# coin-or/Ipopt

Hardware: AMD Instinct MI355X
Metric: KKT factor+solve GFLOP/s (1 numeric LDL^T factorisation + 2 solves per Ipopt iteration) (higher is better)
Workload: dtype f64; 1 GPU; synth_1e6; kkt_dim=1000000, triplet_nnz=20143342, nnz_L=230755000, ordering=nested dissection + minimum-degree leaves (own), supernodes=50052, tree_levels=110, maxfront=3260, num_neg=400000

## Files before the change

### ipopt_amd/csrc/device_view.hip.inc

```
constexpr int FLAG_STRIDE = 32;

typedef double v2d __attribute__((ext_vector_type(2)));
struct DevView {
    const int* sn_colptr; const int* sn_rowptr; const int* sn_rows; const int* rel;
    const int* child_ptr; const int* child_idx; const int* sn_owner; const int* sn_parent; const int* col_owner;
    const long long* panel_off; const long long* cb_off; const long long* minv_off;
    const int* acolptr; const int* apos; const int* arow; const int* acol;
    const int* dup_ptr; const int* dup_src;
    const int* rslot_ptr; const int* rslot_idx; const int* rslot_col; int rslot_len;
    const int* level_sn;
    const FrontMeta* fmeta;
    const int* relinv;
    const GroupLink* gtab;
    const int* tile_tab;
    const ChildMeta* cmeta;
    const int* perm;
    const double* tvals;
    double* aval;
    double* scale;
    double* scale2;
    double* arv;
    unsigned long long* rowmax;
    double* L;
    double* cb;
    double* wbuf;
    double* minv;
    double* dinv; double* doff; int* ptype; int* lperm;
    int4*   fstat;
    double* xw;
    double* cvec;
    double* bw; double* xacc;
    double* gpart;
    double* zb;
    double* ybuf;
    double* arena; const long long* arena_off;
    double* top_rhs; const long long* top_rhs_off;
    double pivtol, pivtol2, small;
    int* colfail;
    int* qstat;
    double* cnorm;
    const ChainLink* chlink; const ChainDesc* chdesc;
    int strace_b;
    unsigned long long* strace;
    const int* chwg_f; const int* chwg_b; const int* chwait; int* sflag_t; int* sflag_dot; double* dpart; v2d* ytag; v2d* xtag;
    int xcd_affine;
    int* apfail;
    int* tcnt;
    double* isg; int* hasis;
    const int* lc_ptr; const LeafLink* lc_link;
    int* sflag_s;
    v2d* cbt; const long long* cbt_off;
    int* sflag_p;
    int* sflag_b; int* sflag_d; int* sepoch;
    int* zpiv;
    int n, nnz_a, nsn, rank;
    int fastpiv;
    double fastu;
    int asm_pull;
    int norestore;
    unsigned long long* dbg;
};

template <int CTRL>
__device__ __forceinline__ double dpp_f64(double x)
{
    int lo = __double2loint(x), hi = __double2hiint(x);
    lo = __builtin_amdgcn_update_dpp(lo, lo, CTRL, 0xF, 0xF, false);
    hi = __builtin_amdgcn_update_dpp(hi, hi, CTRL, 0xF, 0xF, false);
    return __hiloint2double(hi, lo);
}
__device__ __forceinline__ double readlane_f64(double x, int l)
{
    return __hiloint2double(__builtin_amdgcn_readlane(__double2hiint(x), l), __builtin_amdgcn_readlane(__double2loint(x), l));
}
__device__ __forceinline__ double wave_max_all(double x)
{
    x = fmax(x, dpp_f64<0xB1>(x));
    x = fmax(x, dpp_f64<0x4E>(x));
    x = fmax(x, dpp_f64<0x141>(x));
    x = fmax(x, dpp_f64<0x140>(x));
    return fmax(fmax(readlane_f64(x, 0), readlane_f64(x, 16)), fmax(readlane_f64(x, 32), readlane_f64(x, 48)));
}
__device__ __forceinline__ unsigned long long wave_or_all(unsigned long long v)
{
    int lo = (int)(v & 0xffffffffull), hi = (int)(v >> 32);
    lo |= __builtin_amdgcn_update_dpp(lo, lo, 0xB1, 0xF, 0xF, false);  hi |= __builtin_amdgcn_update_dpp(hi, hi, 0xB1, 0xF, 0xF, false);
    lo |= __builtin_amdgcn_update_dpp(lo, lo, 0x4E, 0xF, 0xF, false);  hi |= __builtin_amdgcn_update_dpp(hi, hi, 0x4E, 0xF, 0xF, false);
    lo |= __builtin_amdgcn_update_dpp(lo, lo, 0x141, 0xF, 0xF, false); hi |= __builtin_amdgcn_update_dpp(hi, hi, 0x141, 0xF, 0xF, false);
    lo |= __builtin_amdgcn_update_dpp(lo, lo, 0x140, 0xF, 0xF, false); hi |= __builtin_amdgcn_update_dpp(hi, hi, 0x140, 0xF, 0xF, false);
    const unsigned int l = (unsigned)(__builtin_amdgcn_readlane(lo, 0) | __builtin_amdgcn_readlane(lo, 16) | __builtin_amdgcn_readlane(lo, 32) | __builtin_amdgcn_readlane(lo, 48));
    const unsigned int h = (unsigned)(__builtin_amdgcn_readlane(hi, 0) | __builtin_amdgcn_readlane(hi, 16) | __builtin_amdgcn_readlane(hi, 32) | __builtin_amdgcn_readlane(hi, 48));
    return ((unsigned long long)h << 32) | l;
}
__device__ __forceinline__ double wave_sum_dpp(double x)
{
    x += dpp_f64<0xB1>(x);
    x += dpp_f64<0x4E>(x);
    x += dpp_f64<0x141>(x);
    x += dpp_f64<0x140>(x);
    return (readlane_f64(x, 0) + readlane_f64(x, 16)) + (readlane_f64(x, 32) + readlane_f64(x, 48));
}
__device__ __forceinline__ double wave_sum(double x)
{
#pragma unroll
    for (int off = 32; off >= 1; off >>= 1) x += __shfl_xor(x, off);
    return x;
}
```

### ipopt_amd/csrc/kernels_solve.hip.inc

```
__global__ void k_load_rhs(DevView V, const double* b)
{
    for (int i = blockIdx.x * blockDim.x + threadIdx.x; i < V.n; i += gridDim.x * blockDim.x) V.xw[i] = V.scale[i] * b[V.perm[i]];
}
__global__ void k_store_sol(DevView V, double* b)
{
    for (int i = blockIdx.x * blockDim.x + threadIdx.x; i < V.n; i += gridDim.x * blockDim.x) b[V.perm[i]] = V.scale[i] * V.xw[i];
}

__global__ void k_refine_residual(DevView V, int first)
{
    for (int i = blockIdx.x * blockDim.x + threadIdx.x; i < V.n; i += gridDim.x * blockDim.x)
        V.xacc[i] = first ? V.xw[i] : V.xacc[i] + V.xw[i];
}
__global__ void k_refine_spmv(DevView V)
{
    for (int i = blockIdx.x * blockDim.x + threadIdx.x; i < V.n; i += gridDim.x * blockDim.x) {
        double acc = 0.0;
        for (int p = V.rslot_ptr[i]; p < V.rslot_ptr[i + 1]; ++p) {
            const int q = V.rslot_idx[p];
            const int r = V.arow[q], c = V.acol[q];
            acc += V.aval[q] * V.xacc[r == i ? c : r];
        }
        V.xw[i] = V.bw[i] - acc;
    }
// ... 1147 lines not shown
        flag_raise(&V.sflag_dot[(size_t)(C.dot0 + r) * FLAG_STRIDE], epoch);
        if (tr && tid == 0) tr[3] = wall_clock64();
        return;
    }
    const int jt = r - ndots;
    const int j = C.nlinks - 1 - jt;
    const int nlater = jt;
    const ChainLink Me = uni(V.chlink[C.link0 + j]);
    const int k = Me.k, c0 = Me.c0;
    double mreg[16], lrA[16], lrB[16];
    int lpv = 0;
    auto fetch_block = [&](double (&lr)[16], const int i) {
        const ChainLink L = V.chlink[C.link0 + C.nlinks - 1 - i];
        const double* Lb = V.L + uni(Me.panel_off) + (uni(L.koff) - uni(Me.koff));
        const int kl = uni(L.k);
        const int off = (col < k ? col : 0) * uni(Me.ldp) + part;
#pragma unroll
        for (int u = 0; u < 16; ++u) lr[u] = (col < k && part + 4 * u < kl) ? Lb[off + 4 * u] : 0.0;
    };
    if (!poller) {
        const double* Mg = V.minv + Me.minv_off;
#pragma unroll
        for (int u = 0; u < 16; ++u) { const int q = col + part + 4 * u; mreg[u] = (col < k && q < k) ? Mg[q + (size_t)col * k] : 0.0; }
        if (col < k) lpv = V.lperm[c0 + col];
        if (nlater > 0) fetch_block(lrA, 0);
        if (nlater > 1) fetch_block(lrB, 1);
    } else {
        for (int i = lane; i < min(nlater, 64); i += 64) { const ChainLink L = V.chlink[C.link0 + C.nlinks - 1 - i]; lc0[i] = L.c0; lkk[i] = L.k; }
    }
    const double zv = (tid < k) ? V.zb[c0 + tid] : 0.0;
    if (C.tail > 0) {
        flags_await(V.sflag_dot, nullptr, C.dot0 + jt * nbk, C.dot0 + (jt + 1) * nbk, epoch, err);
        if (tr && tid == 0) tr[1] = wall_clock64();
        if (tid < 64) {
            double t = 0.0;
            const double* dp = V.dpart + (size_t)(C.dot0 + jt * nbk) * 64 + tid;
            for (int b = 0; b < nbk; ++b) t += (tid < k) ? ld_coh(dp + (size_t)b * 64) : 0.0;
            ws[tid] = zv - t;
        }
    } else if (tid < 64) ws[tid] = zv;
    __syncthreads();
    double wv = poller ? 0.0 : ws[col];
    __syncthreads();
    if (tr && tid == 0) tr[2] = wall_clock64();
    auto poll = [&](const int i, double* dst) {
        if ((i & 63) == 0 && i > 0) { for (int q = lane; q < min(nlater - i, 64); q += 64) { const ChainLink L = V.chlink[C.link0 + C.nlinks - 1 - i - q]; lc0[q] = L.c0; lkk[q] = L.k; } __builtin_amdgcn_wave_barrier(); }
        dst[lane] = tag_await(V.xtag + lc0[i & 63], lane, lkk[i & 63], ep, nlater - 1 - i, err);
    };
    auto step = [&](double (&lr)[16], const double* xm, const int i) {
        double a0 = 0.0, a1 = 0.0;
#pragma unroll
        for (int u = 0; u < 16; u += 2) { a0 += lr[u] * xm[part + 4 * u]; a1 += lr[u + 1] * xm[part + 4 * u + 4]; }
        if (i + 2 < nlater) fetch_block(lr, i + 2);
        double t = a0 + a1;
        t += dpp_f64<0xB1>(t); t += dpp_f64<0x4E>(t);
        wv -= t;
    };
    for (int i = 0; i < nlater; i += 2) {
        if (poller) poll(i, xmsg[0]);
        __syncthreads();
        if (!poller) step(lrA, xmsg[0], i);
        if (i + 1 < nlater) {
            if (poller) poll(i + 1, xmsg[1]);
            __syncthreads();
            if (!poller) step(lrB, xmsg[1], i + 1);
        }
    }
    if (poller) return;
    if (part == 0) ws[col] = wv;
    __syncthreads();
    double a0 = 0.0, a1 = 0.0;
#pragma unroll
    for (int u = 0; u < 16; u += 2) { a0 += mreg[u] * ws[(col + part + 4 * u) & 63]; a1 += mreg[u + 1] * ws[(col + part + 4 * u + 4) & 63]; }
    double x = a0 + a1;
    x += dpp_f64<0xB1>(x); x += dpp_f64<0x4E>(x);
    if (part == 0 && col < k) {
        v2d m; m.x = x; m.y = ep;
        st_tag(V.xtag + c0 + lpv, m);
        st_coh(&V.xw[c0 + lpv], x);
    }
    flag_raise(&V.sflag_b[(size_t)Me.fi * FLAG_STRIDE], epoch);
    if (tr && tid == 0) tr[3] = wall_clock64();
}
```

### ipopt_amd/csrc/numeric.hip

```cpp
#include <hip/hip_runtime.h>
#include <rccl/rccl.h>
#include <dlfcn.h>
#include <cstdio>
#include <cstring>
#include <cmath>
#include <chrono>
#include <vector>
#include <thread>
#include <map>
#include <string>
#include <algorithm>
#include "numeric.h"
#include "launch_plan.h"
#include "env_knobs.h"
#include "matching_scaling.h"
#include "device_owner.h"
#include "lowrank_host.h"
#include "lbfgs_host.h"

namespace mi355x {

enum KernelKind { KK_GATHER_SCALE = 0, KK_FRONT_WAVE, KK_FRONT_LDS64, KK_FRONT_LDS128, KK_BIG_ASSEMBLE, KK_BIG_DIAG, KK_BIG_TRSM,
                  KK_BIG_SCHUR, KK_STATS, KK_SOLVE_PERM, KK_FWD_WAVE, KK_FWD_LDS, KK_FWD_BIG, KK_BWD_WAVE, KK_BWD_LDS, KK_BWD_BIG, KK_FWD_BIG_UPD, KK_BWD_BIG_DOT, KK_COUNT };
#define DBGSTAMP(slot) do { if (V.dbg && blockIdx.x == 0 && blockIdx.y == 0 && threadIdx.x == 0) { V.dbg[2 * (slot)] = clock64(); V.dbg[2 * (slot) + 1] = wall_clock64(); } } while (0)
// ... 446 lines not shown
        PlanInputs in = plan_inputs_from_env(opt.nranks, opt.rank, multi, opt.verbose);
        {
            std::vector<long long>& pool_cut = in.pool_cut;
            const long long total = Sy.l_doubles + Sy.cb_doubles;
            long long piece = 1ll << 60;
            if (const char* e = getenv("MI355X_KKT_POOL_PIECE_MIB")) piece = std::max(1ll, atoll(e)) << 17;
            std::vector<long long> starts;
            starts.reserve(2 * (size_t)Sy.num_sn + 1);
            for (int sn = 0; sn < Sy.num_sn; ++sn) if (Sy.alias_child[sn] < 0) { starts.push_back(Sy.panel_off[sn]); starts.push_back(Sy.l_doubles + Sy.cb_off[sn]); }
            starts.push_back(total);
            std::sort(starts.begin(), starts.end());
            long long cur = 0, last_ok = 0;
            pool_cut.push_back(0);
            for (long long b : starts) {
                if (b <= cur) continue;
                while (b - cur > piece && last_ok > cur) { cur = last_ok; pool_cut.push_back(cur); }
                last_ok = b;
            }
            std::vector<char*> base(pool_cut.size(), nullptr);
            if (kept_pool && (pool_cut.size() != 1 || total > kept_pool_doubles)) { own_pool.clear(); kept_pool = nullptr; kept_pool_doubles = 0; }
            for (size_t i = 0; i < pool_cut.size(); ++i) {
                const long long end = i + 1 < pool_cut.size() ? pool_cut[i + 1] : total;
                double* pp = nullptr;
                if (pool_cut.size() == 1 && kept_pool) {
                    pp = kept_pool;
                    HIPCHK(hipMemsetAsync(pp, 0, (size_t)std::max<long long>(total, 1) * sizeof(double), stream));
                } else if (pool_cut.size() == 1) {
                    const long long cap = total + total / 100 + 1024;
                    if (!own_pool.zeroed(&pp, (size_t)cap)) { own_pool.clear(); return false; }
                    kept_pool = pp; kept_pool_doubles = cap;
                } else if (!dalloc(&pp, (size_t)std::max<long long>(end - pool_cut[i], 1))) return false;
                base[i] = (char*)pp;
                in.pool_delta.push_back((long long)((base[i] - base[0]) / (ptrdiff_t)sizeof(double)) - pool_cut[i]);
            }
            V.L = (double*)base[0];
            if (opt.verbose >= 2) fprintf(stderr, "[mi355x_kkt]   pool: %.2f GiB in %zu pieces\n", 8.0 * (double)total / (1024.0 * 1024.0 * 1024.0), pool_cut.size());
        }
        lap("pool");
        knobs = in;
        P = build_launch_plan(Sy, in);
        if (!P.error.empty()) { err_ = P.error; return false; }
        V.fastpiv = in.fastpiv ? 1 : 0; V.asm_pull = in.asm_pull ? 1 : 0; V.fastu = in.fastpiv_floor;
        df_grid_cap = 0;
        if (!P.df_runs.empty()) {
            int per_cu = 0, ncu = 0;
            (void)hipOccupancyMaxActiveBlocksPerMultiprocessor(&per_cu, (const void*)k_front_df, 64, 0);
            (void)hipDeviceGetAttribute(&ncu, hipDeviceAttributeMultiprocessorCount, dev);
            df_grid_cap = std::max(1, per_cu) * std::max(1, ncu);
            if (opt.verbose) { int nl = 0; for (auto& R : P.df_runs) nl += R.nlev; fprintf(stderr, "[mi355x_kkt] small fronts: %d runs covering %d of %d levels in one data-flow launch each (grid <= %d workgroups)\n", (int)P.df_runs.size(), nl, Sy.num_levels, df_grid_cap); }
        }
        lap("host-side schedules and tables");
        if (!upload(P.wgf, &V.chwg_f) || !upload(P.wgb, &V.chwg_b) || !upload(P.chwait, &V.chwait)) return false;
        V.strace = nullptr; V.strace_b = (int)P.wgf.size(); strace_n = 0;
        if (knob_trace("solve") && !P.wgf.empty()) {
            strace_n = 4 * (P.wgf.size() + P.wgb.size());
            if (!dalloc(&V.strace, strace_n)) return false;
            strace_desc.clear();
            for (size_t i = 0; i < P.wgf.size(); ++i) { const ChainDesc& D = P.chd[P.wgf[i]]; strace_desc.push_back({P.wgf[i], (int)i - D.wg0f, D.nlinks, D.tail}); }
            for (size_t i = 0; i < P.wgb.size(); ++i) { const ChainDesc& D = P.chd[P.wgb[i]]; strace_desc.push_back({P.wgb[i], (int)i - D.wg0b - D.nlinks * ((D.tail + 255) / 256), D.nlinks, D.tail}); }
        }
        n_sflag_dot = (size_t)std::max(P.ndots, 1) * FLAG_STRIDE; n_dpart = (size_t)std::max(P.ndots, 1) * 64; n_sflag_t = (size_t)std::max(P.ntailflags, 1) * FLAG_STRIDE; n_sflag_b = std::max<size_t>(P.chl.size(), 1) * FLAG_STRIDE;
        if (!dalloc(&V.sflag_dot, n_sflag_dot) || !dalloc(&V.dpart, n_dpart) || !dalloc(&V.sflag_t, n_sflag_t) || !dalloc(&V.sflag_b, n_sflag_b)) return false;
        n_tag = P.chl.empty() ? 1 : (size_t)Sy.n + 64;
        if (!dalloc(&V.ytag, n_tag) || !dalloc(&V.xtag, n_tag)) return false;
        if (!upload(P.chl, &V.chlink) || !upload(P.chd, &V.chdesc) || !upload(P.tile_tab, &V.tile_tab) || !upload(P.relinv, &V.relinv)) return false;
        if (!dalloc(&V.isg, (size_t)std::max<long long>((long long)P.nbig * ISG_STRIDE, 1)) || !dalloc(&V.hasis, Sy.num_sn)) return false;
        if (!upload(P.fmeta, &V.fmeta) || !upload(P.cmeta, &V.cmeta) || !upload(P.gtab, &V.gtab) || !upload(P.lc_ptr, &V.lc_ptr) || !upload(P.lc_link, &V.lc_link) ||
            !upload(P.df_tab, &d_dftab) || !upload(P.cbt_off, &V.cbt_off) || !dalloc(&V.cbt, (size_t)std::max<long long>(P.cbt_len, 1))) return false;
        const std::vector<long long> moff(Sy.minv_off.begin(), Sy.minv_off.end());
        if (!upload(Sy.sn_colptr, &V.sn_colptr) || !upload(Sy.sn_rowptr, &V.sn_rowptr) || !upload(Sy.sn_rows, &V.sn_rows) ||
            !upload(Sy.rel, &V.rel) || !upload(Sy.child_ptr, &V.child_ptr) || !upload(Sy.child_idx, &V.child_idx) ||
            !upload(P.stat_owner, &V.sn_owner) || !upload(P.panel_off, &V.panel_off) || !upload(P.cb_off, &V.cb_off) || !upload(moff, &V.minv_off) ||
            !upload(Sy.acolptr, &V.acolptr) || !upload(Sy.apos, &V.apos) || !upload(Sy.arow, &V.arow) || !upload(Sy.acol, &V.acol) ||
            !upload(Sy.dup_ptr, &V.dup_ptr) || !upload(Sy.dup_src, &V.dup_src) || !upload(Sy.rslot_ptr, &V.rslot_ptr) || !upload(Sy.rslot_idx, &V.rslot_idx) || !upload(Sy.rslot_col, &V.rslot_col) || !upload(P.lvl_list, &V.level_sn) ||
            !upload(Sy.sn_parent, &V.sn_parent) || !upload(P.col_owner, &V.col_owner) || !upload(P.ex.aoff, &V.arena_off) || !upload(P.ex.troff, &V.top_rhs_off) ||
            !upload(Sy.perm, &V.perm)) return false;
        lap("uploads");
        if (!V.tvals) { double* tv = nullptr; if (!own_handle.zeroed(&tv, Sy.nnz_in)) return false; V.tvals = tv; }
        V.rslot_len = (int)Sy.rslot_idx.size();
        if (!dalloc(&V.arv, Sy.rslot_idx.size()) || !dalloc(&V.aval, Sy.nnz_a) || !dalloc(&V.scale, Sy.n) || !dalloc(&V.scale2, Sy.n) || !dalloc(&V.rowmax, Sy.n) ||
            !dalloc(&V.wbuf, (size_t)Sy.wbuf_doubles) || !dalloc(&V.minv, (size_t)Sy.minv_doubles) ||
            !dalloc(&V.dinv, Sy.n) || !dalloc(&V.doff, Sy.n) || !dalloc(&V.ptype, Sy.n) || !dalloc(&V.lperm, Sy.n) ||
            !dalloc(&V.fstat, Sy.num_sn) || !dalloc(&V.xw, Sy.n) || !dalloc(&V.ybuf, Sy.n) || !dalloc(&V.zb, Sy.n) || !dalloc(&V.bw, Sy.n) || !dalloc(&V.xacc, Sy.n) || !dalloc(&V.cvec, (size_t)Sy.cvec_doubles) || !dalloc(&V.gpart, (size_t)Sy.gpart_doubles) ||
            !dalloc(&d_stats, 12) || !dalloc(&V.colfail, Sy.n) || !dalloc(&V.zpiv, Sy.n) || !dalloc(&V.cnorm, Sy.n) ||
            !dalloc(&V.sflag_d, Sy.num_sn) || !dalloc(&V.sflag_p, Sy.num_sn) || !dalloc(&V.sflag_s, 4 * (size_t)Sy.num_sn) || !dalloc(&V.tcnt, Sy.num_sn) || !dalloc(&V.apfail, Sy.num_sn) || !dalloc(&V.sepoch, 4)) return false;
        V.qstat = d_stats + 4;
        lap("device allocations");
        if (opt.scaling >= 3 && !d_user_scale) { if (!own_handle.raw(&d_user_scale, Sy.n)) return false; }
        else if (opt.scaling == 2 && !d_user_scale) opt.scaling = 1;
        V.cb = V.L + Sy.l_doubles;
        V.arena = nullptr; V.top_rhs = nullptr; V.rank = opt.rank; V.dbg = nullptr;
        if (knob_trace("clocks")) { if (!dalloc(&V.dbg, 128)) return false; }
        if (multi) { if (!dalloc(&V.arena, (size_t)P.ex.arena_doubles) || !dalloc(&V.top_rhs, (size_t)P.ex.toprhs_doubles)) return false; }
        V.pivtol = opt.pivtol; V.pivtol2 = std::max(opt.pivtol, opt.pivtolmax); V.small = opt.small; V.n = Sy.n; V.nnz_a = Sy.nnz_a; V.nsn = Sy.num_sn; V.xcd_affine = knob_disabled("xcd_affine") ? 0 : 1;
        la_ev.assign(1 + P.grp.size(), LaEvents());
        for (size_t i = 0; i < la_ev.size(); ++i) {
            const std::vector<int>& la2 = i == 0 ? P.la_tiles2 : P.grp[i - 1].la2;
            la_ev[i].A.assign(la2.size(), nullptr); la_ev[i].B.assign(la2.size(), nullptr);
            for (size_t lv = 0; lv < la2.size(); ++lv)
                if (la2[lv] > 0 && (!own_struct.event(&la_ev[i].A[lv], hipEventDisableTiming) || !own_struct.event(&la_ev[i].B[lv], hipEventDisableTiming))) return false;
        }
        HIPCHK(hipFuncSetAttribute((const void*)k_big_diag_reg<4>, hipFuncAttributeMaxDynamicSharedMemorySize, 160 * 1024));
        HIPCHK(hipFuncSetAttribute((const void*)(k_big_diag_reg<4, 1024>), hipFuncAttributeMaxDynamicSharedMemorySize, 160 * 1024));
        HIPCHK(hipFuncSetAttribute((const void*)(k_front_reg<64, 2>), hipFuncAttributeMaxDynamicSharedMemorySize, 160 * 1024));
        HIPCHK(hipFuncSetAttribute((const void*)(k_front_reg<64, 4>), hipFuncAttributeMaxDynamicSharedMemorySize, 160 * 1024));
        HIPCHK(hipFuncSetAttribute((const void*)(k_front_reg<64, 8>), hipFuncAttributeMaxDynamicSharedMemorySize, 160 * 1024));
        HIPCHK(hipFuncSetAttribute((const void*)(k_front_reg<256, 8>), hipFuncAttributeMaxDynamicSharedMemorySize, 160 * 1024));
        HIPCHK(hipFuncSetAttribute((const void*)(k_front_reg<256, 6>), hipFuncAttributeMaxDynamicSharedMemorySize, 160 * 1024));
        HIPCHK(hipFuncSetAttribute((const void*)(k_front_reg<256, 8, true>), hipFuncAttributeMaxDynamicSharedMemorySize, 160 * 1024));
        HIPCHK(hipFuncSetAttribute((const void*)(k_front_reg<256, 6, true, 4>), hipFuncAttributeMaxDynamicSharedMemorySize, 160 * 1024));
        HIPCHK(hipFuncSetAttribute((const void*)k_big_trsm<false>, hipFuncAttributeMaxDynamicSharedMemorySize, 160 * 1024));
        HIPCHK(hipFuncSetAttribute((const void*)k_big_trsm<true>, hipFuncAttributeMaxDynamicSharedMemorySize, 160 * 1024));
        HIPCHK(hipFuncSetAttribute((const void*)k_big_diag_trsm, hipFuncAttributeMaxDynamicSharedMemorySize, 160 * 1024));
        HIPCHK(hipFuncSetAttribute((const void*)k_grp_fused, hipFuncAttributeMaxDynamicSharedMemorySize, 160 * 1024));
        HIPCHK(hipFuncSetAttribute((const void*)k_big_assemble2, hipFuncAttributeMaxDynamicSharedMemorySize, 158 * 1024));
        HIPCHK(hipDeviceSynchronize());
        lap("kernel attributes, zero fills landed");
        ready = true;
        if (keep && comm_kind == 2) make_subcomms();
        return true;
    }

    static size_t trsm_lds(int kk) { return trsm_lds_bytes(kk, false); }
    static int schur_grid(int tiles) { return SCHUR_GM == 2 ? 16 * ((tiles + 7) / 8) : tiles; }
    int grid1d(long long n) const { long long g = (n + 255) / 256; return (int)std::min<long long>(std::max<long long>(g, 1), 2048); }


    bool is_single(const Sched& sc) const { return &sc == &P.single; }
    static int bucket0(const Sched& sc, int lv, int fc) { return sc.base + sc.ptr[(size_t)lv * FC_COUNT + fc]; }
    bool launch_bucket(const Sched& sc, int lv, int fc, int top_mode) {
        const int b0 = bucket0(sc, lv, fc), b1 = bucket0(sc, lv, fc + 1), nb = b1 - b0;
        if (nb == 0) return true;
        const bool sg = is_single(sc);
        const size_t rl = P.reg_lds[(size_t)lv * FC_COUNT + fc];
        if (fc == FC_WAVE) {
            const int nt = sg ? P.tiny_split[lv] : 0;
            int fl = top_mode;
            if (V.fastpiv && P.wave_mmin[lv] <= 16) {
                const int n16 = sg ? P.tiny16[lv] : nb;
                if (n16 > 0) { LAUNCH(KK_FRONT_WAVE, k_front_dpp16, dim3((n16 + 3) / 4), dim3(64), 0, stream, V, b0, n16, top_mode, (optimistic && n16 == nb) ? 1 : 0); fl |= 2; }
                if (optimistic && n16 == nb) return true;
            }
            if (nt > 0) LAUNCH(KK_FRONT_WAVE, (k_front_reg<64, 2>), dim3(nt), dim3(64), rl, stream, V, b0, fl);
            if (nb - nt > 0) LAUNCH(KK_FRONT_WAVE, (k_front_reg<64, 4>), dim3(nb - nt), dim3(64), rl, stream, V, b0 + nt, fl);
        } else if (fc == FC_LDS64) {
            LAUNCH(KK_FRONT_LDS64, (k_front_reg<64, 8>), dim3(nb), dim3(64), rl, stream, V, b0, top_mode);
        } else if (fc == FC_LDS128) {
            const int nm = sg ? P.mid_split[lv] : 0;
            const int fl = top_mode | (V.fastpiv ? 2 : 0);
            if (V.fastpiv) {
                if (nm > 0) LAUNCH(KK_FRONT_LDS128, (k_front_reg<256, 6, true, 4>), dim3(nm), dim3(256), P.mid_lds[lv], stream, V, b0, top_mode);
                if (nb - nm > 0) LAUNCH(KK_FRONT_LDS128, (k_front_reg<256, 8, true>), dim3(nb - nm), dim3(256), rl, stream, V, b0 + nm, top_mode);
            }
            if (nm > 0) LAUNCH(KK_FRONT_LDS128, (k_front_reg<256, 6>), dim3(nm), dim3(256), P.mid_lds[lv], stream, V, b0, fl);
            if (nb - nm > 0) LAUNCH(KK_FRONT_LDS128, (k_front_reg<256, 8>), dim3(nb - nm), dim3(256), rl, stream, V, b0 + nm, fl);
        } else {
            const bool single = sg && !multi;
            const int mm = sc.maxm[lv], kk = sc.maxk[lv];
            if ((single || multi) && P.grouped && lv >= S->grp_cut_level) {
                if (!(single && P.lv_asm_skip[lv])) launch_assemble(mm, nb, b0, top_mode);
                return launch_groups(lv, top_mode ? 1 + grp_step : 0);
            }
            if (!single) { const bool sm = mm <= 640; return launch_big(lv, b0, sm ? b1 : b0, b1, top_mode, mm, kk, sm ? sc.tiles64[lv] : 0, sm ? 0 : sc.tiles[lv], false); }
            return launch_big(lv, b0, b0 + P.big_split[lv], b1, top_mode, mm, kk, P.part_tiles[0][lv], P.part_tiles[1][lv], true);
        }
        return true;
    }
// ... 143 lines not shown

    bool norestore_on = !knob_disabled("norestore");
    bool optimistic = false;
    bool optimistic_ok = true;
    int  opt_backoff = 0, opt_wait = 0;
    hipGraphExec_t g_factor_full = nullptr;
    bool factor(const double* dvals, bool reuse, FactorStats& st) {
        DeviceGuard guard(dev);
        if (!ready) { if (err_.empty()) err_ = "factor: solver not set up (no device?)"; return false; }
        if (!from_assembly) { asm_dirty = true; scale_valid = false; }
        if (multi) return factor_dist(dvals, reuse, st);
        ++factor_count;
        static const bool opt_off = knob_disabled("optimistic");
        if (!optimistic_ok && opt_wait > 0 && --opt_wait == 0) optimistic_ok = true;
        optimistic = V.fastpiv && !opt_off && !prof_on && optimistic_ok;
        if (!factor_once(dvals, reuse, st)) return false;
        if (optimistic && (h_stats[8] != 0 || h_stats[9] != 0)) {
            optimistic = false; optimistic_ok = false;
            opt_backoff = opt_backoff == 0 ? 8 : std::min(256, 2 * opt_backoff); opt_wait = opt_backoff;
            if (opt.verbose) fprintf(stderr, h_stats[10] ? "[mi355x_kkt] factor: a wait of the data-flow launch over the small-front levels timed out (device shared?), running the full schedule\n"
                                                           : "[mi355x_kkt] factor: the optimistic schedule met a front for the strict kernels, running the full one\n");
            return factor_once(nullptr, true, st);
        }
        return true;
    }
    bool stage_values(const double* dvals, bool reuse) {
        V.pivtol = opt.pivtol; V.pivtol2 = std::max(opt.pivtol, opt.pivtolmax); V.small = opt.small;
        if (!reuse) {
            if (dvals) HIPCHK(hipMemcpyAsync((void*)V.tvals, dvals, S->nnz_in * sizeof(double), hipMemcpyDeviceToDevice, stream));
            else       HIPCHK(hipMemcpyAsync((void*)V.tvals, h_vals, S->nnz_in * sizeof(double), hipMemcpyHostToDevice, stream));
            have_values = true;
        } else if (!have_values) { err_ = "refactor: no values on the device yet"; return false; }
        if (want_matching() && S->n > 0) { if (!run_matching()) return false; match_valid = true; }
        HIPCHK(hipEventRecord(ev0, stream));
        return true;
    }
    bool finish_timed(double& timer, bool add = false, void* hdst = nullptr, const void* dsrc = nullptr, size_t bytes = 0) {
        HIPCHK(hipEventRecord(ev1, stream));
        if (bytes) HIPCHK(hipMemcpyAsync(hdst, dsrc, bytes, hipMemcpyDeviceToHost, stream));
        HIPCHK(hipStreamSynchronize(stream));
        float ms = 0; HIPCHK(hipEventElapsedTime(&ms, ev0, ev1)); timer = add ? timer + ms : ms;
        return true;
    }
    void read_factor_stats(FactorStats& st) const {
        st.num_neg = h_stats[0]; st.num_zero = h_stats[1]; st.num_two = h_stats[2]; st.num_small = h_stats[3]; st.u_sensitive = h_stats[4] != 0; st.num_fast = h_stats[7];
    }
    template <class F> bool capture_into(hipGraphExec_t& exec, F enqueue) {
        hipGraph_t g = nullptr;
        HIPCHK(hipStreamBeginCapture(stream, hipStreamCaptureModeThreadLocal));
        const bool ok = enqueue();
        const hipError_t e = hipStreamEndCapture(stream, &g);
        if (!ok) return false;
        if (e != hipSuccess) { err_ = std::string("hipStreamEndCapture: ") + hipGetErrorString(e); return false; }
        HIPCHK(hipGraphInstantiate(&exec, g, nullptr, nullptr, 0));
        (void)hipGraphDestroy(g);
        return true;
    }
    bool factor_once(const double* dvals, bool reuse, FactorStats& st) {
        V.norestore = (optimistic && norestore_on) ? 1 : 0;
        if (!stage_values(dvals, reuse)) return false;
        if (opt.use_graph && !P.la_any) {
            if (graph_pivtol != V.pivtol || graph_pivtol2 != V.pivtol2) {
                destroy_factor_graphs();
            }
            hipGraphExec_t& g_factor = keep_scale_now ? (optimistic ? g_factor_keep : g_factor_full_keep) : (optimistic ? this->g_factor : g_factor_full);
            if (!g_factor) {
                if (!capture_into(g_factor, [&] { return enqueue_factor(); })) return false;
                graph_pivtol = V.pivtol; graph_pivtol2 = V.pivtol2;
                HIPCHK(hipEventRecord(ev0, stream));
            }
            HIPCHK(hipGraphLaunch(g_factor, stream));
        } else {
            if (!enqueue_factor()) return false;
        }
        if (!keep_scale_now && opt.scaling == 1) scale_valid = true;
        if (!finish_timed(factor_ms, false, h_stats, d_stats, 12 * sizeof(int))) return false;
        read_factor_stats(st);
        if (h_stats[5] != 0) { err_ = "factor: a panel workgroup timed out waiting for its pivot block"; return false; }
        return true;
    }
    double graph_pivtol = -1.0, graph_pivtol2 = -1.0;

    const bool mid_on = !knob_disabled("mid_solve");
    static size_t lds_solve(int mmax, int kmax) { return (size_t)(mmax + 3 * kmax) * sizeof(double) + 16; }
    void solve_level(const Sched& sc, int lv, bool forward, int top_mode) {
        const bool single = is_single(sc), pair = single && P.pair_solve, mid = single && !top_mode && mid_on && S->maxsupernode <= MID_KMAX;
        for (int fc = 0; fc < FC_COUNT; ++fc) {
            const int b0 = bucket0(sc, lv, fc), nb = bucket0(sc, lv, fc + 1) - b0;
            if (nb == 0) continue;
            const int g0 = sc.last0[lv], ng = sc.last1[lv] - g0, mm = sc.maxm[lv];
            if (forward) {
                if (fc == FC_WAVE && pair && P.wave_mmax[lv] <= 16) LAUNCH(KK_FWD_WAVE, (k_fwd_pair<16, 16>), dim3((nb + 3) / 4), dim3(64), 0, stream, V, b0, nb);
                else if (fc == FC_WAVE && pair && P.wave_kmax[lv] <= 16) LAUNCH(KK_FWD_WAVE, (k_fwd_pair<16>), dim3((nb + 1) / 2), dim3(64), 0, stream, V, b0, nb);
                else if (fc == FC_WAVE && pair) LAUNCH(KK_FWD_WAVE, (k_fwd_pair<32>), dim3((nb + 1) / 2), dim3(64), 0, stream, V, b0, nb);
                else if (fc == FC_WAVE)   LAUNCH(KK_FWD_WAVE, (k_fwd<64>),  dim3(nb), dim3(64),  lds_solve(32, 32),   stream, V, b0, top_mode);
                else if (fc == FC_LDS64 && mid)  LAUNCH(KK_FWD_LDS,  (k_fwd_mid<1>), dim3(nb), dim3(64), 0, stream, V, b0);
                else if (fc == FC_LDS128 && mid) LAUNCH(KK_FWD_LDS,  (k_fwd_mid<2>), dim3(nb), dim3(64), 0, stream, V, b0);
                else if (fc == FC_LDS64)  LAUNCH(KK_FWD_LDS,  (k_fwd<64>),  dim3(nb), dim3(64),  lds_solve(64, 64),   stream, V, b0, top_mode);
                else if (fc == FC_LDS128) LAUNCH(KK_FWD_LDS,  (k_fwd<256>), dim3(nb), dim3(256), lds_solve(128, 128), stream, V, b0, top_mode);
                else if (ng <= 0) continue;
                else if (single && sc.allsolo[lv] && sc.maxk[lv] <= 64) LAUNCH(KK_FWD_BIG, k_fwd_solo64, dim3((mm + 63) / 64 + 1, ng), dim3(256), 0, stream, V, g0);
                else if ((single || !top_mode) && sc.allsolo[lv]) LAUNCH(KK_FWD_BIG, k_fwd_solo, dim3((mm + 63) / 64 + 1, ng), dim3(256), 0, stream, V, g0);
                else { LAUNCH(KK_FWD_BIG, k_fwd_grp, dim3(ng), dim3(256), 0, stream, V, g0, top_mode);
                       LAUNCH(KK_FWD_BIG_UPD, k_fwd_grp_upd, dim3((mm + 63) / 64, ng), dim3(256), 0, stream, V, g0); }
            } else {
                if (fc == FC_WAVE && pair && P.wave_mmax[lv] <= 16) LAUNCH(KK_BWD_WAVE, (k_bwd_pair<16, 16>), dim3((nb + 3) / 4), dim3(64), 0, stream, V, b0, nb);
                else if (fc == FC_WAVE && pair && P.wave_kmax[lv] <= 16) LAUNCH(KK_BWD_WAVE, (k_bwd_pair<16>), dim3((nb + 1) / 2), dim3(64), 0, stream, V, b0, nb);
                else if (fc == FC_WAVE && pair) LAUNCH(KK_BWD_WAVE, (k_bwd_pair<32>), dim3((nb + 1) / 2), dim3(64), 0, stream, V, b0, nb);
                else if (fc == FC_WAVE)   LAUNCH(KK_BWD_WAVE, (k_bwd<64>),  dim3(nb), dim3(64),  lds_solve(32, 32),   stream, V, b0);
                else if (fc == FC_LDS64 && mid)  LAUNCH(KK_BWD_LDS,  (k_bwd_mid<1>), dim3(nb), dim3(64), 0, stream, V, b0);
                else if (fc == FC_LDS128 && mid) LAUNCH(KK_BWD_LDS,  (k_bwd_mid<2>), dim3(nb), dim3(64), 0, stream, V, b0);
                else if (fc == FC_LDS64)  LAUNCH(KK_BWD_LDS,  (k_bwd<64>),  dim3(nb), dim3(64),  lds_solve(64, 64),   stream, V, b0);
                else if (fc == FC_LDS128) LAUNCH(KK_BWD_LDS,  (k_bwd<256>), dim3(nb), dim3(256), lds_solve(128, 128), stream, V, b0);
                else if (ng <= 0) continue;
                else if (single && !S->solve_group && sc.maxk[lv] <= 64) {
                    LAUNCH(KK_BWD_BIG_DOT, k_bwd_dot64, dim3((mm + 255) / 256, ng), dim3(256), 0, stream, V, g0);
                    LAUNCH(KK_BWD_BIG, k_bwd_fin64, dim3(ng), dim3(256), 0, stream, V, g0);
                } else {
                    LAUNCH(KK_BWD_BIG_DOT, k_bwd_grp_dot, dim3((mm + 255) / 256, ng), dim3(256), 0, stream, V, g0);
                    LAUNCH(KK_BWD_BIG, k_bwd_grp, dim3(ng), dim3(256), 0, stream, V, g0); }
            }
        }
    }
    bool solve_sweep(const Sched& sc, bool forward, int top_mode, bool use_segs = true) {
        const int NL = S->num_levels;
        const bool single = is_single(sc), segs = single || (top_mode && use_segs);
        int lcs = (single && P.pair_solve && P.lc_levels > 0) ? P.lc_levels : 0;
        for (int lv = 0; lv < lcs; ++lv) if (P.seg_at_lv0[lv] >= 0) { lcs = 0; break; }
        if (forward && lcs > 0) LAUNCH(KK_FWD_WAVE, k_fwd_leafchain, dim3((P.lc_nchains + 3) / 4), dim3(64), 0, stream, V, P.lc_nchains);
        for (int q = lcs; q < NL; ++q) {
            const int lv = forward ? q : NL - 1 + lcs - q;
            const int sgi = !segs ? -1 : forward ? P.seg_at_lv0[lv] : P.seg_at_lv1[lv];
            if (sgi < 0) { solve_level(sc, lv, forward, top_mode); continue; }
            const ChainSeg& sg = P.chain_segs[sgi];
            if (forward) {
                if (single && gate_on && !gate_entered) { if (gate_valid) HIPCHK(hipStreamWaitEvent(stream, gate_last, 0)); gate_entered = true; }
                LAUNCH(KK_FWD_BIG, k_fwd_chain, dim3(sg.nwg_f), dim3(320), 0, stream, V, sg.wgf0);
            } else {
                LAUNCH(KK_BWD_BIG, k_bwd_chain, dim3(sg.nwg_b), dim3(320), 0, stream, V, sg.wgb0);
                if (single && gate_on && gate_mine) { HIPCHK(hipEventRecord(gate_mine, stream)); gate_last = gate_mine; gate_valid = true; }
            }
            q += sg.lv1 - sg.lv0;
        }
        if (!forward && lcs > 0) LAUNCH(KK_BWD_WAVE, k_bwd_leafchain, dim3((P.lc_nchains + 3) / 4), dim3(64), 0, stream, V, P.lc_nchains);
        HIPCHK(hipGetLastError());
        return true;
    }

    bool enqueue_solve(const double* dsrc, double* drhs) {
        LAUNCH(KK_SOLVE_PERM, k_load_rhs, dim3(grid1d(S->n)), dim3(256), 0, stream, V, dsrc);
        if (!enqueue_solve_core()) return false;
        LAUNCH(KK_SOLVE_PERM, k_store_sol, dim3(grid1d(S->n)), dim3(256), 0, stream, V, drhs);
        HIPCHK(hipGetLastError());
        return true;
    }
    bool enqueue_solve_core() {
        const int n = S->n;
        const int nref = opt.refine_steps > 0 ? opt.refine_steps : 0;
        if (nref > 0) LAUNCH(KK_SOLVE_PERM, k_save_rhs, dim3(grid1d(n)), dim3(256), 0, stream, V);
        for (int pass = 0; pass <= nref; ++pass) {
            if (pass > 0) {
                LAUNCH(KK_SOLVE_PERM, k_refine_residual, dim3(grid1d(n)), dim3(256), 0, stream, V, pass == 1 ? 1 : 0);
                LAUNCH(KK_SOLVE_PERM, k_refine_spmv, dim3(grid1d(n)), dim3(256), 0, stream, V);
            }
            if (!P.chain_segs.empty()) LAUNCH(KK_SOLVE_PERM, k_bump_epoch, dim3(1), dim3(64), 0, stream, V.sepoch);
            if (!solve_sweep(P.single, true, 0) || !solve_sweep(P.single, false, 0)) return false;
        }
        if (nref > 0) LAUNCH(KK_SOLVE_PERM, k_refine_finish, dim3(grid1d(n)), dim3(256), 0, stream, V);
        HIPCHK(hipGetLastError());
        return true;
    }

    static constexpr int SOLVE_CTX = 3;
    struct SolveCtx { hipStream_t strm = nullptr; hipEvent_t done = nullptr; hipGraphExec_t graph = nullptr;
                      double *xw = nullptr, *cvec = nullptr, *bw = nullptr, *xacc = nullptr, *gpart = nullptr, *zb = nullptr, *ybuf = nullptr, *dpart = nullptr;
                      int *sflag_t = nullptr, *sflag_dot = nullptr, *sflag_b = nullptr, *sepoch = nullptr; v2d *ytag = nullptr, *xtag = nullptr; };
    SolveCtx sctx[SOLVE_CTX]; int nsctx = 1; hipEvent_t sctx_fork = nullptr;
    int sctx_verdict = 0; bool sctx_tuning = false;
    bool gate_on = false, gate_valid = false, gate_entered = false; hipEvent_t gate_last = nullptr, gate_mine = nullptr; hipEvent_t gate_ev[SOLVE_CTX] = {nullptr, nullptr, nullptr};
    size_t n_sflag_dot = 1, n_dpart = 1, n_sflag_t = 1, n_sflag_b = 1, n_tag = 1;
    void sctx_release() {
        for (hipEvent_t& e : gate_ev) e = nullptr;
        gate_on = gate_valid = gate_entered = false; gate_last = gate_mine = nullptr; sctx_verdict = 0;
        for (int c = 1; c < SOLVE_CTX; ++c) { if (sctx[c].graph) (void)hipGraphExecDestroy(sctx[c].graph); if (sctx[c].strm) (void)hipStreamDestroy(sctx[c].strm); sctx[c] = SolveCtx(); }
        sctx_fork = nullptr; nsctx = 1;
    }
    bool sctx_ensure(int want) {
        want = std::min(want, SOLVE_CTX);
        const Symbolic& Sy = *S;
        if (!sctx_fork && !own_struct.event(&sctx_fork, hipEventDisableTiming)) return false;
        for (int c = 0; c < want; ++c) if (!gate_ev[c] && !own_struct.event(&gate_ev[c], hipEventDisableTiming)) return false;
        for (int c = nsctx; c < want; ++c) {
            SolveCtx& X = sctx[c];
            { int plo = 0, phi = 0; (void)hipDeviceGetStreamPriorityRange(&plo, &phi);
              HIPCHK(hipStreamCreateWithPriority(&X.strm, hipStreamNonBlocking, c == 1 ? (plo + phi) / 2 : plo)); }
            if (!own_struct.event(&X.done, hipEventDisableTiming)) return false;
            if (!dalloc(&X.xw, Sy.n) || !dalloc(&X.ybuf, Sy.n) || !dalloc(&X.zb, Sy.n) || !dalloc(&X.bw, Sy.n) || !dalloc(&X.xacc, Sy.n) || !dalloc(&X.cvec, (size_t)Sy.cvec_doubles) ||
                !dalloc(&X.gpart, (size_t)Sy.gpart_doubles) || !dalloc(&X.sflag_dot, n_sflag_dot) || !dalloc(&X.dpart, n_dpart) || !dalloc(&X.sflag_t, n_sflag_t) || !dalloc(&X.sflag_b, n_sflag_b) ||
                !dalloc(&X.ytag, n_tag) || !dalloc(&X.xtag, n_tag) || !dalloc(&X.sepoch, 4)) return false;
            HIPCHK(hipDeviceSynchronize());
            nsctx = c + 1;
        }
        return true;
    }
    void sctx_swap(int c) {
        SolveCtx& X = sctx[c];
        std::swap(stream, X.strm); std::swap(g_solve, X.graph);
        std::swap(V.xw, X.xw); std::swap(V.cvec, X.cvec); std::swap(V.bw, X.bw); std::swap(V.xacc, X.xacc); std::swap(V.gpart, X.gpart); std::swap(V.zb, X.zb); std::swap(V.ybuf, X.ybuf);
        std::swap(V.dpart, X.dpart); std::swap(V.sflag_t, X.sflag_t); std::swap(V.sflag_dot, X.sflag_dot); std::swap(V.sflag_b, X.sflag_b); std::swap(V.sepoch, X.sepoch);
        std::swap(V.ytag, X.ytag); std::swap(V.xtag, X.xtag);
    }
    bool solve_one(const double* src, double* col) {
        if (opt.use_graph) {
            if (!g_solve && !capture_into(g_solve, [&] { return enqueue_solve_core(); })) return false;
            hipLaunchKernelGGL(k_load_rhs, dim3(grid1d(S->n)), dim3(256), 0, stream, V, src);
            HIPCHK(hipGraphLaunch(g_solve, stream));
            hipLaunchKernelGGL(k_store_sol, dim3(grid1d(S->n)), dim3(256), 0, stream, V, col);
            return true;
        }
        return enqueue_solve(src, col);
    }
    bool solve_device(int nrhs, const double* dsrc, int lds_, double* drhs, int ld, bool timed) {
        DeviceGuard guard(dev);
        if (!ready) { if (err_.empty()) err_ = "solve: solver not set up"; return false; }
        if (multi) return solve_dist(nrhs, dsrc, lds_, drhs, ld);
        if (timed) HIPCHK(hipEventRecord(ev0, stream));
        int nctx = (nrhs > 1 && !prof_on && !V.strace && !knob_disabled("solve_ctx")) ? std::min(nrhs, SOLVE_CTX) : 1;
        if (nctx > 1 && sctx_verdict == 0 && !sctx_tuning) {
            DeviceOwner tune(err_);
            double* scratch = nullptr;
            if (!tune.raw(&scratch, 6 * (size_t)std::max(S->n, 1))) return false;
            HIPCHK(hipMemsetAsync(scratch, 0, 6 * (size_t)std::max(S->n, 1) * sizeof(double), stream));
            sctx_tuning = true;
            float t_seq = 0, t_ctx = 0; bool ok = true;
            hipEvent_t e0 = nullptr, e1 = nullptr; if (!tune.event(&e0) || !tune.event(&e1)) return false;
            for (int mode = 0; mode < 2 && ok; ++mode) {
                sctx_verdict = mode == 0 ? 2 : 1;
                float best = 1e30f;
                for (int rep = 0; rep < 4 && ok; ++rep) {
                    HIPCHK(hipEventRecord(e0, stream));
                    ok = solve_device(3, scratch, S->n, scratch + 3 * (size_t)S->n, S->n, false);
                    HIPCHK(hipEventRecord(e1, stream)); HIPCHK(hipStreamSynchronize(stream));
                    float ms = 0; if (ok) HIPCHK(hipEventElapsedTime(&ms, e0, e1));
                    if (rep > 0) best = std::min(best, ms);
                }
                (mode == 0 ? t_seq : t_ctx) = best;
            }
            tune.clear();
            sctx_tuning = false;
            if (!ok) { sctx_verdict = 0; return false; }
            sctx_verdict = t_ctx < 0.95f * t_seq ? 1 : 2;
            if (opt.verbose) fprintf(stderr, "[mi355x_kkt] solve contexts for nrhs > 1: three right-hand sides %.3f ms one after the other, %.3f ms through the contexts -> %s\n", t_seq, t_ctx, sctx_verdict == 1 ? "contexts" : "one after the other");
            if (timed) HIPCHK(hipEventRecord(ev0, stream));
        }
        if (sctx_verdict == 2 && !knob_int("solve_ctx_force", 0)) nctx = 1;
        if (nctx > 1) {
            if (!sctx_ensure(nctx)) return false;
            HIPCHK(hipEventRecord(sctx_fork, stream));
            for (int c = 1; c < nctx; ++c) HIPCHK(hipStreamWaitEvent(sctx[c].strm, sctx_fork, 0));
            gate_on = true; gate_valid = false;
            bool ok = true;
            for (int r = 0; r < nrhs && ok; ++r) {
                const int c = r % nctx;
                double* col = drhs + (size_t)r * ld;
                const double* src = dsrc + (size_t)r * lds_;
                gate_mine = gate_ev[c]; gate_entered = false;
                if (c > 0) sctx_swap(c);
                ok = enqueue_solve(src, col);
                if (c > 0) sctx_swap(c);
            }
            gate_on = false; gate_mine = nullptr;
            if (!ok) return false;
            for (int c = 1; c < nctx; ++c) {
                HIPCHK(hipEventRecord(sctx[c].done, sctx[c].strm)); HIPCHK(hipStreamWaitEvent(stream, sctx[c].done, 0));
                if (!P.chain_segs.empty()) hipLaunchKernelGGL(k_merge_err, dim3(1), dim3(64), 0, stream, V.sepoch + 1, (const int*)(sctx[c].sepoch + 1));
            }
        } else
            for (int r = 0; r < nrhs; ++r) if (!solve_one(dsrc + (size_t)r * lds_, drhs + (size_t)r * ld)) return false;
        if (timed) {
            if (!finish_timed(solve_ms, false, h_stats + 6, V.sepoch + 1, P.chain_segs.empty() ? 0 : sizeof(int))) return false;
            if (V.strace) {
                std::vector<unsigned long long> h(strace_n);
                HIPCHK(hipMemcpy(h.data(), V.strace, strace_n * sizeof(unsigned long long), hipMemcpyDeviceToHost));
                std::string trace_path; knob_trace("solve", &trace_path);
                if (FILE* f = fopen(trace_path.c_str(), "w")) {
                    for (size_t i = 0; i < strace_desc.size(); ++i)
                        fprintf(f, "%c %d %d %d %d %llu %llu %llu %llu\n", i < (size_t)V.strace_b ? 'F' : 'B', strace_desc[i].chain, strace_desc[i].w, strace_desc[i].nlinks, strace_desc[i].tail,
                                h[4 * i], h[4 * i + 1], h[4 * i + 2], h[4 * i + 3]);
                    fclose(f);
                }
            }
// ... 739 lines not shown
```

Before: 9953 GFLOP/s.

## Fuse big-front backward dot and finish via last-block ticket; merge small LDS buckets

Adds k_bwd_big64, which computes the panel dot-product partials for a big front with k≤64. The last chunk block to finish, found through a per-front atomic ticket, reduces the partials and applies Minv in the same kernel. This replaces the separate k_bwd_dot64 + k_bwd_fin64 launches with one launch per level. It also lets sparse LDS64 fronts ride along in the LDS128 launch when they are few, saving another launch. The cost is per-context ticket buffers and atomics, and cross-block coherence now depends on the ticket ordering.

```diff
diff --git a/ipopt_amd/csrc/device_view.hip.inc b/ipopt_amd/csrc/device_view.hip.inc
--- a/ipopt_amd/csrc/device_view.hip.inc
+++ b/ipopt_amd/csrc/device_view.hip.inc
@@ -31,6 +31,7 @@
     double* cvec;
     double* bw; double* xacc;
     double* gpart;
+    int* bticket;
     double* zb;
     double* ybuf;
     double* arena; const long long* arena_off;
diff --git a/ipopt_amd/csrc/kernels_solve.hip.inc b/ipopt_amd/csrc/kernels_solve.hip.inc
--- a/ipopt_amd/csrc/kernels_solve.hip.inc
+++ b/ipopt_amd/csrc/kernels_solve.hip.inc
@@ -1253,3 +1253,84 @@
     flag_raise(&V.sflag_b[(size_t)Me.fi * FLAG_STRIDE], epoch);
     if (tr && tid == 0) tr[3] = wall_clock64();
 }
+
+
+__global__ __launch_bounds__(256) void k_bwd_big64(DevView V, int list_off)
+{
+    __shared__ double pl[64], ws[64];
+    __shared__ int tks;
+    const int unit = list_off + blockIdx.y;
+    const FrontMeta M = V.fmeta[unit];
+    const int tid = threadIdx.x, lane = tid & 63, wave = tid >> 6;
+    const int k = M.k, c0 = M.c0;
+    const int nch = (M.m - k + 255) / 256;
+    if ((int)blockIdx.x >= (nch > 1 ? nch : 1)) return;
+    const int ibase = k + blockIdx.x * 256;
+    const int nrow = min(256, M.m - ibase);
+    const bool v0 = lane < nrow, v1 = lane + 64 < nrow, v2 = lane + 128 < nrow, v3 = lane + 192 < nrow;
+    const double* Lg = V.L + M.panel_off + ibase + lane;
+    double lv[4][4][4];
+#pragma unroll
+    for (int ps = 0; ps < 4; ++ps)
+#pragma unroll
+        for (int u = 0; u < 4; ++u) {
+            const int col = wave * 4 + 16 * ps + u;
+            const bool cv = col < k;
+            const double* c = Lg + (size_t)col * M.ldp;
+            lv[ps][u][0] = (cv && v0) ? c[0] : 0.0; lv[ps][u][1] = (cv && v1) ? c[64] : 0.0;
+            lv[ps][u][2] = (cv && v2) ? c[128] : 0.0; lv[ps][u][3] = (cv && v3) ? c[192] : 0.0;
+        }
+    const double zbv = tid < k ? V.zb[c0 + tid] : 0.0;
+    const int pcol = tid >> 2, part4 = tid & 3;
+    const int lpv = (part4 == 0 && pcol < k) ? V.lperm[c0 + pcol] : 0;
+    const int r0i = M.r0 + ibase;
+    const double x0 = v0 ? V.xw[V.sn_rows[r0i + lane]] : 0.0, x1 = v1 ? V.xw[V.sn_rows[r0i + lane + 64]] : 0.0;
+    const double x2 = v2 ? V.xw[V.sn_rows[r0i + lane + 128]] : 0.0, x3 = v3 ? V.xw[V.sn_rows[r0i + lane + 192]] : 0.0;
+    double* part = V.gpart + M.gpart + (size_t)blockIdx.x * M.gcols;
+#pragma unroll
+    for (int ps = 0; ps < 4; ++ps)
+#pragma unroll
+        for (int u = 0; u < 4; ++u) {
+            const int col = wave * 4 + 16 * ps + u;
+            double t = (lv[ps][u][0] * x0 + lv[ps][u][1] * x1) + (lv[ps][u][2] * x2 + lv[ps][u][3] * x3);
+            t = wave_sum(t);
+            if (lane == 0 && col < k) { if (nch <= 1) pl[col] = t; else st_coh(part + col, t); }
+        }
+    const double* Mg = V.minv + M.minv_off;
+    double mreg[16];
+#pragma unroll
+    for (int u = 0; u < 16; ++u) { const int q = pcol + part4 + 4 * u; mreg[u] = (pcol < k && q < k) ? Mg[q + (size_t)pcol * k] : 0.0; }
+    if (nch > 1) {
+        asm volatile("s_waitcnt vmcnt(0)" ::: "memory");
+        __syncthreads();
+        if (tid == 0) {
+            const int tk = __hip_atomic_fetch_add(V.bticket + unit, 1, __ATOMIC_RELAXED, __HIP_MEMORY_SCOPE_AGENT);
+            if (tk == nch - 1) st_coh(V.bticket + unit, 0);
+            tks = tk;
+        }
+        __syncthreads();
+        if (tks != nch - 1) return;
+    } else __syncthreads();
+    if (tid < 64) {
+        double w = 0.0;
+        if (tid < k) {
+            const double* pg = V.gpart + M.gpart;
+            double t0 = 0.0, t1 = 0.0, t2 = 0.0, t3 = 0.0;
+            if (nch == 1) t0 += pl[tid];
+            else {
+                int c = 0;
+                for (; c + 3 < nch; c += 4) { t0 += ld_coh(pg + (size_t)c * M.gcols + tid); t1 += ld_coh(pg + (size_t)(c + 1) * M.gcols + tid);
+                                              t2 += ld_coh(pg + (size_t)(c + 2) * M.gcols + tid); t3 += ld_coh(pg + (size_t)(c + 3) * M.gcols + tid); }
+                for (; c < nch; ++c) t0 += ld_coh(pg + (size_t)c * M.gcols + tid);
+            }
+            w = zbv - ((t0 + t1) + (t2 + t3));
+        }
+        ws[tid] = w;
+    }
+    __syncthreads();
+    double a = 0.0;
+#pragma unroll
+    for (int u = 0; u < 16; ++u) a += mreg[u] * ws[(pcol + part4 + 4 * u) & 63];
+    a += __shfl_xor(a, 1); a += __shfl_xor(a, 2);
+    if (part4 == 0 && pcol < k) V.xw[c0 + lpv] = a;
+}
diff --git a/ipopt_amd/csrc/numeric.hip b/ipopt_amd/csrc/numeric.hip
--- a/ipopt_amd/csrc/numeric.hip
+++ b/ipopt_amd/csrc/numeric.hip
@@ -552,7 +552,7 @@
             !dalloc(&V.wbuf, (size_t)Sy.wbuf_doubles) || !dalloc(&V.minv, (size_t)Sy.minv_doubles) ||
             !dalloc(&V.dinv, Sy.n) || !dalloc(&V.doff, Sy.n) || !dalloc(&V.ptype, Sy.n) || !dalloc(&V.lperm, Sy.n) ||
             !dalloc(&V.fstat, Sy.num_sn) || !dalloc(&V.xw, Sy.n) || !dalloc(&V.ybuf, Sy.n) || !dalloc(&V.zb, Sy.n) || !dalloc(&V.bw, Sy.n) || !dalloc(&V.xacc, Sy.n) || !dalloc(&V.cvec, (size_t)Sy.cvec_doubles) || !dalloc(&V.gpart, (size_t)Sy.gpart_doubles) ||
-            !dalloc(&d_stats, 12) || !dalloc(&V.colfail, Sy.n) || !dalloc(&V.zpiv, Sy.n) || !dalloc(&V.cnorm, Sy.n) ||
+            !dalloc(&V.bticket, n_bticket = std::max<size_t>(P.fmeta.size(), 1)) || !dalloc(&d_stats, 12) || !dalloc(&V.colfail, Sy.n) || !dalloc(&V.zpiv, Sy.n) || !dalloc(&V.cnorm, Sy.n) ||
             !dalloc(&V.sflag_d, Sy.num_sn) || !dalloc(&V.sflag_p, Sy.num_sn) || !dalloc(&V.sflag_s, 4 * (size_t)Sy.num_sn) || !dalloc(&V.tcnt, Sy.num_sn) || !dalloc(&V.apfail, Sy.num_sn) || !dalloc(&V.sepoch, 4)) return false;
         V.qstat = d_stats + 4;
         lap("device allocations");
@@ -862,12 +862,17 @@
     double graph_pivtol = -1.0, graph_pivtol2 = -1.0;
 
     const bool mid_on = !knob_disabled("mid_solve");
+    const bool big_on = !knob_disabled("big_solve");
     static size_t lds_solve(int mmax, int kmax) { return (size_t)(mmax + 3 * kmax) * sizeof(double) + 16; }
     void solve_level(const Sched& sc, int lv, bool forward, int top_mode) {
         const bool single = is_single(sc), pair = single && P.pair_solve, mid = single && !top_mode && mid_on && S->maxsupernode <= MID_KMAX;
+        const bool big1 = single && !top_mode && big_on && !S->solve_group && sc.maxk[lv] <= 64;
+        const int n64 = bucket0(sc, lv, FC_LDS64 + 1) - bucket0(sc, lv, FC_LDS64), n128 = bucket0(sc, lv, FC_LDS128 + 1) - bucket0(sc, lv, FC_LDS128);
+        const bool ride = mid && big_on && n64 > 0 && 8 * n64 <= n128;
         for (int fc = 0; fc < FC_COUNT; ++fc) {
-            const int b0 = bucket0(sc, lv, fc), nb = bucket0(sc, lv, fc + 1) - b0;
-            if (nb == 0) continue;
+            int b0 = bucket0(sc, lv, fc), nb = bucket0(sc, lv, fc + 1) - b0;
+            if (nb == 0 || (ride && fc == FC_LDS64)) continue;
+            if (ride && fc == FC_LDS128) { b0 -= n64; nb += n64; }
             const int g0 = sc.last0[lv], ng = sc.last1[lv] - g0, mm = sc.maxm[lv];
             if (forward) {
                 if (fc == FC_WAVE && pair && P.wave_mmax[lv] <= 16) LAUNCH(KK_FWD_WAVE, (k_fwd_pair<16, 16>), dim3((nb + 3) / 4), dim3(64), 0, stream, V, b0, nb);
@@ -893,6 +898,7 @@
                 else if (fc == FC_LDS64)  LAUNCH(KK_BWD_LDS,  (k_bwd<64>),  dim3(nb), dim3(64),  lds_solve(64, 64),   stream, V, b0);
                 else if (fc == FC_LDS128) LAUNCH(KK_BWD_LDS,  (k_bwd<256>), dim3(nb), dim3(256), lds_solve(128, 128), stream, V, b0);
                 else if (ng <= 0) continue;
+                else if (big1) LAUNCH(KK_BWD_BIG_DOT, k_bwd_big64, dim3(std::max((mm + 255) / 256, 1), ng), dim3(256), 0, stream, V, g0);
                 else if (single && !S->solve_group && sc.maxk[lv] <= 64) {
                     LAUNCH(KK_BWD_BIG_DOT, k_bwd_dot64, dim3((mm + 255) / 256, ng), dim3(256), 0, stream, V, g0);
                     LAUNCH(KK_BWD_BIG, k_bwd_fin64, dim3(ng), dim3(256), 0, stream, V, g0);
@@ -954,11 +960,11 @@
     static constexpr int SOLVE_CTX = 3;
     struct SolveCtx { hipStream_t strm = nullptr; hipEvent_t done = nullptr; hipGraphExec_t graph = nullptr;
                       double *xw = nullptr, *cvec = nullptr, *bw = nullptr, *xacc = nullptr, *gpart = nullptr, *zb = nullptr, *ybuf = nullptr, *dpart = nullptr;
-                      int *sflag_t = nullptr, *sflag_dot = nullptr, *sflag_b = nullptr, *sepoch = nullptr; v2d *ytag = nullptr, *xtag = nullptr; };
+                      int *bticket = nullptr, *sflag_t = nullptr, *sflag_dot = nullptr, *sflag_b = nullptr, *sepoch = nullptr; v2d *ytag = nullptr, *xtag = nullptr; };
     SolveCtx sctx[SOLVE_CTX]; int nsctx = 1; hipEvent_t sctx_fork = nullptr;
     int sctx_verdict = 0; bool sctx_tuning = false;
     bool gate_on = false, gate_valid = false, gate_entered = false; hipEvent_t gate_last = nullptr, gate_mine = nullptr; hipEvent_t gate_ev[SOLVE_CTX] = {nullptr, nullptr, nullptr};
-    size_t n_sflag_dot = 1, n_dpart = 1, n_sflag_t = 1, n_sflag_b = 1, n_tag = 1;
+    size_t n_sflag_dot = 1, n_dpart = 1, n_sflag_t = 1, n_sflag_b = 1, n_tag = 1, n_bticket = 1;
     void sctx_release() {
         for (hipEvent_t& e : gate_ev) e = nullptr;
         gate_on = gate_valid = gate_entered = false; gate_last = gate_mine = nullptr; sctx_verdict = 0;
@@ -976,7 +982,7 @@
               HIPCHK(hipStreamCreateWithPriority(&X.strm, hipStreamNonBlocking, c == 1 ? (plo + phi) / 2 : plo)); }
             if (!own_struct.event(&X.done, hipEventDisableTiming)) return false;
             if (!dalloc(&X.xw, Sy.n) || !dalloc(&X.ybuf, Sy.n) || !dalloc(&X.zb, Sy.n) || !dalloc(&X.bw, Sy.n) || !dalloc(&X.xacc, Sy.n) || !dalloc(&X.cvec, (size_t)Sy.cvec_doubles) ||
-                !dalloc(&X.gpart, (size_t)Sy.gpart_doubles) || !dalloc(&X.sflag_dot, n_sflag_dot) || !dalloc(&X.dpart, n_dpart) || !dalloc(&X.sflag_t, n_sflag_t) || !dalloc(&X.sflag_b, n_sflag_b) ||
+                !dalloc(&X.gpart, (size_t)Sy.gpart_doubles) || !dalloc(&X.bticket, n_bticket) || !dalloc(&X.sflag_dot, n_sflag_dot) || !dalloc(&X.dpart, n_dpart) || !dalloc(&X.sflag_t, n_sflag_t) || !dalloc(&X.sflag_b, n_sflag_b) ||
                 !dalloc(&X.ytag, n_tag) || !dalloc(&X.xtag, n_tag) || !dalloc(&X.sepoch, 4)) return false;
             HIPCHK(hipDeviceSynchronize());
             nsctx = c + 1;
@@ -986,7 +992,7 @@
     void sctx_swap(int c) {
         SolveCtx& X = sctx[c];
         std::swap(stream, X.strm); std::swap(g_solve, X.graph);
-        std::swap(V.xw, X.xw); std::swap(V.cvec, X.cvec); std::swap(V.bw, X.bw); std::swap(V.xacc, X.xacc); std::swap(V.gpart, X.gpart); std::swap(V.zb, X.zb); std::swap(V.ybuf, X.ybuf);
+        std::swap(V.xw, X.xw); std::swap(V.cvec, X.cvec); std::swap(V.bw, X.bw); std::swap(V.xacc, X.xacc); std::swap(V.gpart, X.gpart); std::swap(V.bticket, X.bticket); std::swap(V.zb, X.zb); std::swap(V.ybuf, X.ybuf);
         std::swap(V.dpart, X.dpart); std::swap(V.sflag_t, X.sflag_t); std::swap(V.sflag_dot, X.sflag_dot); std::swap(V.sflag_b, X.sflag_b); std::swap(V.sepoch, X.sepoch);
         std::swap(V.ytag, X.ytag); std::swap(V.xtag, X.xtag);
     }
```

After: 10010 GFLOP/s, median of 6. About the same (+0.6%).
